# MPF-Optimization-Laboratory/ConicIP.jl

Hardware: NVIDIA B200
Metric: kkt_factor_plus_solves_per_sec (higher is better)
Workload: dtype f64

## Files before the change

conicip.jl_b200/csrc/engine.h:

```cpp
#pragma once
#include <vector>

#include "../../include/conicip_b200.h"
#include "kernels.cuh"

constexpr int NV = 8;
constexpr int MV = 10;
constexpr int PV = 6;

namespace cip {
struct Multi;

struct RowStructure {
  bool on = false;
  int nsing = 0, nempty = 0, nr = 0, nr_pad = 0, nJ = 0, nJ_pad = 0;
  bool compressed = false, base_has_gtg = false, fold = false;
  double *At4r = nullptr, *Atil4r = nullptr, *Hr4 = nullptr;
  double* Base4 = nullptr;
  GemmOperand map{};
  int *rest_row = nullptr, *J = nullptr, *Jinv = nullptr;
  int* row_code = nullptr;
  int *sing_ptr = nullptr, *sing_row = nullptr, *sing_col = nullptr;
  double* sing_val = nullptr;
  ConeDesc cd{};
  int *d_type = nullptr, *d_off = nullptr, *d_rowcone = nullptr, *d_qlist = nullptr, *d_slist = nullptr;
  int* cone_map = nullptr;
  Scaling Fi{};
  double *xr[2] = {}, *yJ[2] = {}, *outr[2] = {}, *outJ[2] = {};

  struct Split {
    bool on = false;
    int nK = 0, nK_pad = 0, from_rest = 0, from_Q = 0, from_G = 0;
    bool g_in_D = false;
    bool factored = false;
    std::vector<int> K;
    std::vector<char> q_couple;
    struct QEntry { int i, j; double v; };
    std::vector<QEntry> qtrip;
    int *dK = nullptr, *Kpos = nullptr, *JK = nullptr;
    double *QK4 = nullptr, *BaseK4 = nullptr, *HK4 = nullptr, *WinvK = nullptr;
    double *qD = nullptr, *hD = nullptr, *kscale = nullptr;
    double *GK4 = nullptr, *ZK4 = nullptr;
    CholPlan chol{};
    GemmOperand mapZK{}, mapG{};
    int* fail = nullptr;
    double* kv[2][3] = {};
  } sp;
};

struct FastSyrk {
  bool on = false;
  int depth = 0;
  int leaf = 0;
  int K2 = 0;
  unsigned two = 0;
  int nchunk = 0;
  int* colexp = nullptr;
  double* colss = nullptr;
  double* M = nullptr;
  double* M2 = nullptr;
  int4* table = nullptr;
};
}

struct cip_engine {
  cip::Multi* multi = nullptr;
  cip::Multi* parent = nullptr;
  int shard_index = 0;
  bool always_sync = false;
  int n = 0, m = 0, p = 0, n_pad = 0, m_pad = 0, p_pad = 0, ncones = 0;
  int device = 0;
  cudaStream_t stream = nullptr, own_stream = nullptr;
  cip_options opt{};
  double *At4 = nullptr, *Atil4 = nullptr, *Qq4 = nullptr, *H4 = nullptr, *Winv = nullptr;
  double *G4 = nullptr, *Z4 = nullptr, *S4 = nullptr, *Sbase4 = nullptr, *WinvS = nullptr;
  cip::GemmOperand mapAtil{}, mapZ{};
  cip::CholPlan cholH{}, cholS{};
  int* info = nullptr;
  std::vector<int> h_type, h_off;
  int *d_type = nullptr, *d_off = nullptr, *d_rowcone = nullptr, *d_qlist = nullptr, *d_slist = nullptr;
  int *d_sord = nullptr, *d_roff = nullptr;
  double* d_sws = nullptr;
  std::vector<int> h_slist, h_sord, h_roff;
  size_t r_total = 0;
  cip::ConeDesc cd{};
  cip::Scaling F{}, Fi{};
  bool have_scaling = false, have_factor = false;
  double* gemm_ws = nullptr;
  bool fold = false;
  cip::GemmOperand mapAt{};
  int aug_rows = 0;
  double aug_rho = 0.0;
  cip::RowStructure rs;
  cip::FastSyrk fast;
  std::vector<void*> owned;
  double* nv[NV] = {};
  double* mv[MV] = {};
  double* pv[PV] = {};
  double* nv2[6] = {};
  double* mv2[6] = {};
  double* pv2[5] = {};
  double* partial = nullptr;
  int partial_cap = 0;
  double* scalar = nullptr;
  void* comm = nullptr;
  int nranks = 1, rank = 0;
  double* Hp = nullptr;
  cudaStream_t cs = nullptr, s2 = nullptr;
  cudaEvent_t evc[16] = {};
  cip_stats_t st{};
  cudaEvent_t ev[8] = {};
  size_t bytes = 0;
  bool need_sync = false;
};


namespace cip {
int engine_allreduce(cip_engine* h, double* buf, size_t count);
int engine_create_single(cip_handle* out, int n, int m, int p, const double* Q, int ldq, const double* A, int lda,
                         const double* G, int ldg, const cip_csc* Qs, const cip_csc* As, const cip_csc* Gs,
                         int ncones, const int* cone_type, const int* cone_dim, const cip_options* opts);
const char* last_error_string();
int engine_decide_fold(cip_engine* h, bool can, size_t mn, bool* fold);
int engine_setup_comm(cip_engine* h);

int fast_syrk_plan(cip_engine* h, bool can);
size_t fast_syrk_atil_doubles(const cip_engine* h);
int fast_syrk_setup(cip_engine* h);
int fast_syrk_drop(cip_engine* h);
int fast_syrk_form(cip_engine* h, const double* cin);

int structure_build_dense(cip_engine* h);
int structure_build_csc(cip_engine* h, const cip_csc* A);
int structure_finish(cip_engine* h);
int structure_form_H(cip_engine* h);
int structure_AT(cip_engine* h, double* out, const double* x, const double* add, int b);
int structure_AT2(cip_engine* h, double* outa, double* outb, const double* xa, const double* xb, const double* adda,
                  const double* addb);
int structure_A(cip_engine* h, double* out, const double* y, int b);
int structure_A2(cip_engine* h, double* outa, double* outb, const double* ya, const double* yb);
int split_classify_csc_Q(cip_engine* h, const cip_csc* Q);
int split_diag_Q(cip_engine* h, const double* q);
int split_build(cip_engine* h);
int split_factor(cip_engine* h);
int split_add_delta(cip_engine* h, double delta);
int split_solve(cip_engine* h, double** nv, double** pv, int b, bool schur);
int split_mul_Q(cip_engine* h, double* y, const double* x);
int split_get_H(cip_engine* h, double* tmp);

int multi_create(cip_handle* out, int n, int m, int p, const double* Q, int ldq, const double* A, int lda,
                 const double* G, int ldg, const cip_csc* Qs, const cip_csc* As, const cip_csc* Gs, int ncones,
                 const int* cone_type, const int* cone_dim, const cip_options* opts);
int multi_destroy(cip_engine* h);
int multi_factor(cip_engine* h, const int* kind, const double* fa, const double* fb, const double* fD,
                 const double* fR, int factor);
int multi_get_scaling(cip_engine* h, int* kind, double* fa, double* fb, double* fD, double* fR);
int multi_nt_scaling(cip_engine* h, const double* v, const double* s, double* lambda_out, int factor);
int multi_solve(cip_engine* h, const double* ry, const double* rw, const double* rv, double* dy, double* dw,
                double* dv);
int multi_solve_multi(cip_engine* h, int nrhs, const double* ry, int ldy, const double* rw, int ldw, const double* rv,
                      int ldv, double* dy, double* dw, double* dv);
int multi_apply(cip_engine* h, int op, const double* x, double* y);
int multi_maxstep(cip_engine* h, const double* x, const double* d, double d_scale, double* alpha_out);
int multi_prod_div(cip_engine* h, const double* x, const double* y, double* o, int divide);
int multi_mul_A(cip_engine* h, int trans, const double* x, double* y);
int multi_mul_GQ(cip_engine* h, int which, int trans, const double* x, double* y);
int multi_ipm_solve(cip_engine* h, const double* c, const double* b, const double* d, const cip_ipm_options* opts,
                    double* y, double* w, double* v, cip_ipm_result* result);
int multi_stats(cip_engine* h, cip_stats_t* out);
int multi_simple(cip_engine* h, int what, double* out, int ldo);
void multi_barrier(cip::Multi* m);
}
```

conicip.jl_b200/csrc/fast_syrk.cu:

```cuda
#include <stdlib.h>

#include <algorithm>
#include <vector>

#include "engine.h"

namespace cip {

namespace {

constexpr int FAST_SYRK_LEAF = 2048;
constexpr int FAST_SYRK_N0 = 12288;
constexpr int FAST_SYRK_L2_MIN = 1024;

struct SumsArgs {
  int h, kqh, pstride, count;
  int a_row, a_kq, b_row, b_kq, s_row, s_kq, t_row, t_kq;
  int scale_a, scale_b;
};

__device__ __forceinline__ void winograd_sums(double* __restrict__ X, int ld, const SumsArgs& s,
                                              const int* __restrict__ colexp) {
  const int kq = blockIdx.x;
  const int x = blockIdx.y * blockDim.x + threadIdx.x;
  if (x >= s.count) return;
  const int h = s.h, KQ2 = s.kqh;
  const int p = x / h, i = x - p * h, base = p * s.pstride;
  const int xa = base + s.a_row + i, xb = base + s.b_row + i;
  const int ka = s.a_kq + kq, kb = s.b_kq + kq;
  auto at = [&](int kqq, int r) { return reinterpret_cast<double2*>(X + ((size_t)kqq * ld + r) * 4); };
  auto ld4 = [&](int kqq, int r, double f, double2& lo, double2& hi) {
    const double2* q = at(kqq, r);
    lo = q[0]; hi = q[1];
    lo.x *= f; lo.y *= f; hi.x *= f; hi.y *= f;
  };
  auto fac = [&](int on, int r) { return on ? ldexp(1.0, -colexp[r]) : 1.0; };
  const double fa1 = fac(s.scale_a, xa), fa2 = fac(s.scale_a, xa + h);
  const double fb1 = fac(s.scale_b, xb), fb2 = fac(s.scale_b, xb + h);
  double2 a11l, a11h, a12l, a12h, a21l, a21h, a22l, a22h, b11l, b11h, b12l, b12h, b21l, b21h, b22l, b22h;
  ld4(ka, xa, fa1, a11l, a11h);
  ld4(ka + KQ2, xa, fa1, a12l, a12h);
  ld4(ka, xa + h, fa2, a21l, a21h);
  ld4(ka + KQ2, xa + h, fa2, a22l, a22h);
  ld4(kb, xb, fb1, b11l, b11h);
  ld4(kb + KQ2, xb, fb1, b12l, b12h);
  ld4(kb, xb + h, fb2, b21l, b21h);
  ld4(kb + KQ2, xb + h, fb2, b22l, b22h);
  auto add = [](double2 u, double2 v) { return make_double2(u.x + v.x, u.y + v.y); };
  auto sub = [](double2 u, double2 v) { return make_double2(u.x - v.x, u.y - v.y); };
  const double2 s1l = add(a21l, a22l), s1h = add(a21h, a22h);
  const double2 s2l = sub(s1l, a11l), s2h = sub(s1h, a11h);
  const double2 s3l = sub(a11l, a21l), s3h = sub(a11h, a21h);
  const double2 s4l = sub(a12l, s2l), s4h = sub(a12h, s2h);
  const double2 t1l = sub(b21l, b11l), t1h = sub(b21h, b11h);
  const double2 t2l = sub(b22l, t1l), t2h = sub(b22h, t1h);
  const double2 t3l = sub(b22l, b21l), t3h = sub(b22h, b21h);
  const double2 t4l = sub(t2l, b12l), t4h = sub(t2h, b12h);
  const int ks = s.s_kq + kq, kt = s.t_kq + kq, rs = base + s.s_row + i, rt = base + s.t_row + i;
  auto st4 = [&](int kqq, int r, double2 lo, double2 hi) { double2* q = at(kqq, r); q[0] = lo; q[1] = hi; };
  st4(ks, rs, s1l, s1h);
  st4(ks, rs + h, s2l, s2h);
  st4(ks, rs + 2 * h, s3l, s3h);
  st4(ks, rs + 3 * h, s4l, s4h);
  st4(kt, rt, t1l, t1h);
  st4(kt, rt + h, t2l, t2h);
  st4(kt, rt + 2 * h, t3l, t3h);
  st4(kt, rt + 3 * h, t4l, t4h);
}

__global__ void __launch_bounds__(256)
winograd_sums_kernel(double* __restrict__ X, int ld, const SumsArgs s, const int* __restrict__ colexp) {
  winograd_sums(X, ld, s, colexp);
}
__global__ void __launch_bounds__(256)
winograd_sums2_kernel(double* __restrict__ X, int ld, const SumsArgs s, const int* __restrict__ colexp) {
  winograd_sums(X, ld, s, colexp);
}

__global__ void __launch_bounds__(256)
winograd_combine2_kernel(const double* __restrict__ M2, double* __restrict__ M, int h2, int q, int pstride,
                         int x_row, int y_row, int raw_x, int raw_y, const int* __restrict__ colexp) {
  const int nt2 = h2 / TILE, G2 = nt2 * nt2, nt = 2 * nt2, G = nt * nt;
  const int L2 = blockIdx.x, p = blockIdx.y;
  const int ti = L2 % nt2, tj = L2 / nt2;
  const int xr = p * pstride + x_row, yr = p * pstride + y_row;
  const size_t slab = (size_t)TILE * TILE;
  const double* Mp = M2 + ((size_t)p * 7 * G2 + L2) * slab;
  double* Mq = M + (size_t)(p * 7 + q) * G * slab;
  for (int e = threadIdx.x * 2; e < TILE * TILE; e += 512) {
    const int quad = e / (TILE * 4), lr = (e % (TILE * 4)) >> 2, c = e & 3;
    const int i = ti * TILE + lr, j = tj * TILE + quad * 4 + c;
    double2 P[7];
#pragma unroll
    for (int r = 0; r < 7; ++r) P[r] = *reinterpret_cast<const double2*>(Mp + (size_t)r * G2 * slab + e);
    const int ex1 = raw_x ? colexp[xr + i] : 0, ex2 = raw_x ? colexp[xr + h2 + i] : 0;
    const int ey1[2] = {raw_y ? colexp[yr + j] : 0, raw_y ? colexp[yr + j + 1] : 0};
    const int ey2[2] = {raw_y ? colexp[yr + h2 + j] : 0, raw_y ? colexp[yr + h2 + j + 1] : 0};
    double o[4][2];
#pragma unroll
    for (int k = 0; k < 2; ++k) {
      const double p1 = k ? P[0].y : P[0].x, p2 = k ? P[1].y : P[1].x, p3 = k ? P[2].y : P[2].x;
      const double p4 = k ? P[3].y : P[3].x, p5 = k ? P[4].y : P[4].x, p6 = k ? P[5].y : P[5].x;
      const double p7 = k ? P[6].y : P[6].x;
      const double s1 = ldexp(p1, -(ex1 + ey1[k])), s2 = ldexp(p2, -(ex1 + ey1[k]));
      const double u2 = s1 + p6;
      const double u3 = u2 + p7, u4 = u2 + p5;
      o[0][k] = s1 + s2;
      o[1][k] = u4 + ldexp(p3, -ey2[k]);
      o[2][k] = u3 - ldexp(p4, -ex2);
      o[3][k] = u3 + p5;
    }
#pragma unroll
    for (int b = 0; b < 4; ++b) {
      const int L = (ti + (b >> 1) * nt2) + (tj + (b & 1) * nt2) * nt;
      *reinterpret_cast<double2*>(Mq + (size_t)L * slab + e) = make_double2(o[b][0], o[b][1]);
    }
  }
}

__global__ void __launch_bounds__(256)
winograd_combine_kernel(const double* __restrict__ M, const double* __restrict__ Cin, double* __restrict__ H, int ld,
                        int h, int scaled, const int* __restrict__ colexp) {
  const int nt = h / TILE, G = nt * nt;
  const int L = blockIdx.x, p = blockIdx.y;
  const int ti = L % nt, tj = L / nt;
  const int ra = 4 * p * h, rb = ra + 2 * h;
  const size_t slab = (size_t)TILE * TILE;
  const double* Mp = M + ((size_t)p * 7 * G + L) * slab;
  for (int e = threadIdx.x * 2; e < TILE * TILE; e += 512) {
    const int quad = e / (TILE * 4), lr = (e % (TILE * 4)) >> 2, c = e & 3;
    const int i = ti * TILE + lr, j = tj * TILE + quad * 4 + c;
    double2 P[7];
#pragma unroll
    for (int q = 0; q < 7; ++q) P[q] = *reinterpret_cast<const double2*>(Mp + (size_t)q * G * slab + e);
    const int eb1 = colexp[rb + i], eb2 = colexp[rb + h + i];
    const int ea1[2] = {colexp[ra + j], colexp[ra + j + 1]};
    const int ea2[2] = {colexp[ra + h + j], colexp[ra + h + j + 1]};
    double o[4][2];
#pragma unroll
    for (int k = 0; k < 2; ++k) {
      const double p1 = k ? P[0].y : P[0].x, p2 = k ? P[1].y : P[1].x, p3 = k ? P[2].y : P[2].x;
      const double p4 = k ? P[3].y : P[3].x, p5 = k ? P[4].y : P[4].x, p6 = k ? P[5].y : P[5].x;
      const double p7 = k ? P[6].y : P[6].x;
      const double u2 = (scaled ? p1 : ldexp(p1, -(eb1 + ea1[k]))) + p6;
      const double u3 = u2 + p7, u4 = u2 + p5;
      o[0][k] = scaled ? ldexp(p1 + p2, eb1 + ea1[k]) : p1 + p2;
      o[1][k] = ldexp(u4 + (scaled ? p3 : ldexp(p3, -ea2[k])), eb1 + ea2[k]);
      o[2][k] = ldexp(u3 - (scaled ? p4 : ldexp(p4, -eb2)), eb2 + ea1[k]);
      o[3][k] = ldexp(u3 + p5, eb2 + ea2[k]);
    }
#pragma unroll
    for (int b = 0; b < 4; ++b) {
      const size_t idx = q4_index(rb + (b >> 1) * h + i, ra + (b & 1) * h + j, ld);
      double2 v = make_double2(o[b][0], o[b][1]);
      if (Cin) {
        const double2 q = *reinterpret_cast<const double2*>(Cin + idx);
        v.x += q.x;
        v.y += q.y;
      }
      *reinterpret_cast<double2*>(H + idx) = v;
    }
  }
}

int env_int(const char* name, int dflt) {
  const char* e = getenv(name);
  return (e && *e) ? atoi(e) : dflt;
}

template <typename T>
int falloc(cip_engine* h, T** p, size_t count) {
  *p = nullptr;
  if (count == 0) count = 1;
  CIP_CUDA(cudaMalloc(reinterpret_cast<void**>(p), count * sizeof(T)));
  CIP_CUDA(cudaMemsetAsync(*p, 0, count * sizeof(T), h->stream));
  h->bytes += count * sizeof(T);
  h->owned.push_back(*p);
  return 0;
}

size_t m_doubles(int n_pad) { return (size_t)7 * n_pad / 4 * n_pad / 4; }

size_t m2_doubles(int n_pad, unsigned two) {
  if (!two) return 0;
  int d = 0;
  while (!(two >> d & 1u)) ++d;
  const size_t h2 = (size_t)n_pad >> (d + 3);
  return (size_t)7 * ((size_t)1 << d) * h2 * h2;
}

size_t atil_rows(const FastSyrk& f) { return (size_t)4 * f.K2 + (f.two ? f.K2 / 2 : 0); }

void winograd_ops(int4 ops[7], int xr, int xk, int yr, int yk, int hh, int kqh, int sr, int sk, int tr, int tk) {
  ops[0] = make_int4(xr, xk, yr, yk);
  ops[1] = make_int4(xr, xk + kqh, yr, yk + kqh);
  ops[2] = make_int4(sr + 3 * hh, sk, yr + hh, yk + kqh);
  ops[3] = make_int4(xr + hh, xk + kqh, tr + 3 * hh, tk);
  ops[4] = make_int4(sr, sk, tr, tk);
  ops[5] = make_int4(sr + hh, sk, tr + hh, tk);
  ops[6] = make_int4(sr + 2 * hh, sk, tr + 2 * hh, tk);
}

void level1_ops(int4 ops[7], int p, int hh, int KQ2) {
  const int ra = 4 * p * hh, rb = ra + 2 * hh;
  winograd_ops(ops, rb, 0, ra, 0, hh, KQ2, ra, 2 * KQ2, ra, 3 * KQ2);
}

void level2_ops(int4 ops[7], int4 o, int p, int hh, int KQ2) {
  const int ra = 4 * p * hh;
  winograd_ops(ops, o.x, o.y, o.z, o.w, hh / 2, KQ2 / 2, ra, 4 * KQ2, ra + 2 * hh, 4 * KQ2);
}

}

int fast_syrk_plan(cip_engine* h, bool can) {
  FastSyrk& f = h->fast;
  f = FastSyrk{};
  const int mode = env_int("CIP_FAST_SYRK", 2);
  if (!can || mode == 0 || h->m_pad == 0) return 0;
  int leaf = std::max(256, env_int("CIP_FAST_SYRK_LEAF", FAST_SYRK_LEAF));
  if (mode == 1) leaf = std::min(leaf, h->n_pad / 2);
  int W = h->n_pad, depth = 0;
  while (W % 512 == 0 && W / 2 >= leaf) { W /= 2; ++depth; }
  if (depth == 0 || (mode != 1 && h->n_pad < FAST_SYRK_N0)) return 0;
  const int levels = env_int("CIP_FAST_SYRK_LEVELS", 0);
  unsigned two = 0;
  for (int d = 0; d < depth && levels != 1; ++d) {
    const int h2 = h->n_pad >> (d + 3);
    if (h2 % TILE == 0 && (h2 >= FAST_SYRK_L2_MIN || levels == 2)) two |= 1u << d;
  }
  const size_t nn = (size_t)h->n_pad * h->n_pad;
  const size_t colss = (size_t)scale_panel_norms_chunks(h->m_pad) * h->n_pad;
  for (;; two = 0) {
    f.two = two;
    f.K2 = round_up(h->m_pad, two ? 128 : 64) / 2;
    if (mode == 1) break;
    size_t free_b = 0, total_b = 0;
    CIP_CUDA(cudaMemGetInfo(&free_b, &total_b));
    const size_t need = (atil_rows(f) * h->n_pad + m_doubles(h->n_pad) + m2_doubles(h->n_pad, two) + colss + 3 * nn +
                         (size_t)GEMM_WS_DOUBLES) * 8 + (size_t(1) << 30);
    if (free_b >= need) break;
    if (!two) { f = FastSyrk{}; return 0; }
  }
  f.on = true;
  f.depth = depth;
  f.leaf = W;
  f.nchunk = scale_panel_norms_chunks(h->m_pad);
  return 0;
}

size_t fast_syrk_atil_doubles(const cip_engine* h) { return atil_rows(h->fast) * h->n_pad; }

int fast_syrk_setup(cip_engine* h) {
  FastSyrk& f = h->fast;
  if (!f.on) return 0;
  CIP_TRY(falloc(h, &f.colexp, h->n_pad));
  CIP_TRY(falloc(h, &f.colss, (size_t)f.nchunk * h->n_pad));
  CIP_TRY(falloc(h, &f.M, m_doubles(h->n_pad)));
  if (f.two) CIP_TRY(falloc(h, &f.M2, m2_doubles(h->n_pad, f.two)));
  const int KQ2 = f.K2 / 4;
  std::vector<int4> t;
  for (int l = 0; l < (1 << f.depth); ++l) {
    const int r0 = l * f.leaf;
    t.push_back(make_int4(r0, 0, r0, 0));
    t.push_back(make_int4(r0, r0, 0, 0));
  }
  int4 ops[7], sub[7];
  for (int d = 0; d < f.depth; ++d) {
    const int hh = h->n_pad >> (d + 2);
    for (int p = 0; p < (1 << d); ++p) {
      level1_ops(ops, p, hh, KQ2);
      for (const int4& o : ops) {
        t.push_back(o);
        t.push_back(make_int4(0, 0, 0, 0));
      }
    }
  }
  for (int d = 0; d < f.depth; ++d) {
    if (!(f.two >> d & 1u)) continue;
    const int hh = h->n_pad >> (d + 2);
    for (int q = 0; q < 7; ++q)
      for (int p = 0; p < (1 << d); ++p) {
        level1_ops(ops, p, hh, KQ2);
        level2_ops(sub, ops[q], p, hh, KQ2);
        for (const int4& o : sub) {
          t.push_back(o);
          t.push_back(make_int4(0, 0, 0, 0));
        }
      }
  }
  CIP_TRY(falloc(h, &f.table, t.size()));
  CIP_CUDA(cudaMemcpyAsync(f.table, t.data(), t.size() * sizeof(int4), cudaMemcpyHostToDevice, h->stream));
  CIP_CUDA(cudaStreamSynchronize(h->stream));
  return 0;
}

int fast_syrk_drop(cip_engine* h) {
  FastSyrk& f = h->fast;
  if (!f.on) return 0;
  CIP_CUDA(cudaStreamSynchronize(h->stream));
  for (void* p : {(void*)f.colexp, (void*)f.colss, (void*)f.M, (void*)f.M2, (void*)f.table}) {
    if (!p) continue;
    h->owned.erase(std::find(h->owned.begin(), h->owned.end(), p));
    CIP_CUDA(cudaFree(p));
  }
  CIP_CUDA(cudaFree(h->Atil4));
  h->bytes -= fast_syrk_atil_doubles(h) * 8;
  const size_t mn = (size_t)h->m_pad * h->n_pad;
  CIP_CUDA(cudaMalloc(reinterpret_cast<void**>(&h->Atil4), mn * 8));
  CIP_CUDA(cudaMemsetAsync(h->Atil4, 0, mn * 8, h->stream));
  h->bytes += mn * 8;
  CIP_TRY(make_q4_tensor_map(&h->mapAtil.map, h->Atil4, h->n_pad, h->m_pad / 4));
  f = FastSyrk{};
  return 0;
}

int fast_syrk_form(cip_engine* h, const double* cin) {
  const FastSyrk& f = h->fast;
  cudaStream_t s = h->stream;
  const int KQ2 = f.K2 / 4, L = 1 << f.depth;
  int sub_entry = L + 7 * (L - 1);
  for (int d = 0; d < f.depth; ++d) {
    const int pairs = 1 << d, hh = h->n_pad >> (d + 2), nt = hh / TILE;
    const bool two = f.two >> d & 1u;
    SumsArgs sa{hh, KQ2, 4 * hh, pairs * hh, 2 * hh, 0, 0, 0, 0, 2 * KQ2, 0, 3 * KQ2, 1, 1};
    winograd_sums_kernel<<<dim3(KQ2, (sa.count + 255) / 256), 256, 0, s>>>(h->Atil4, h->n_pad, sa, f.colexp);
    CIP_CHECK_LAUNCH();
    GemmArgs g{};
    g.lower = 0; g.ntm = g.ntn = nt; g.sym = 0;
    g.nk = f.K2 / 32;
    g.Ctm = f.M; g.ldc = h->n_pad; g.alpha = 1.0;
    g.ws = h->gemm_ws; g.ws_doubles = GEMM_WS_DOUBLES;
    g.group = f.table + 2 * (L + 7 * (pairs - 1));
    g.group_tiles = nt * nt;
    g.tile_count = 7 * pairs * nt * nt;
    if (!two) {
      CIP_TRY(launch_gemm_nt(h->mapAtil, h->mapAtil, g, s));
    } else {
      const int h2 = hh / 2, nt2 = h2 / TILE;
      int4 ops[7];
      level1_ops(ops, 0, hh, KQ2);
      for (int q = 0; q < 7; ++q) {
        const int4 o = ops[q];
        const int raw_x = o.y < 2 * KQ2, raw_y = o.w < 2 * KQ2;
        SumsArgs s2{h2, KQ2 / 2, 4 * hh, pairs * h2, o.x, o.y, o.z, o.w, 0, 4 * KQ2, 2 * hh, 4 * KQ2, raw_x, raw_y};
        winograd_sums2_kernel<<<dim3(KQ2 / 2, (s2.count + 255) / 256), 256, 0, s>>>(h->Atil4, h->n_pad, s2, f.colexp);
        CIP_CHECK_LAUNCH();
        GemmArgs g2 = g;
        g2.ntm = g2.ntn = nt2;
        g2.nk = f.K2 / 64;
        g2.Ctm = f.M2;
        g2.group = f.table + 2 * sub_entry;
        g2.group_tiles = nt2 * nt2;
        g2.tile_count = 7 * pairs * nt2 * nt2;
        sub_entry += 7 * pairs;
        CIP_TRY(launch_gemm_nt(h->mapAtil, h->mapAtil, g2, s));
        winograd_combine2_kernel<<<dim3(nt2 * nt2, pairs), 256, 0, s>>>(f.M2, f.M, h2, q, 4 * hh, o.x, o.z, raw_x,
                                                                        raw_y, f.colexp);
        CIP_CHECK_LAUNCH();
      }
    }
    winograd_combine_kernel<<<dim3(nt * nt, pairs), 256, 0, s>>>(f.M, cin, h->H4, h->n_pad, hh, two, f.colexp);
    CIP_CHECK_LAUNCH();
  }
  const int T = f.leaf / TILE;
  GemmArgs a{};
  a.lower = 1; a.ntm = a.ntn = T; a.sym = 1;
  a.nk = h->m_pad / 32;
  a.Cin = cin; a.Cout = h->H4; a.ldc = h->n_pad; a.alpha = 1.0;
  a.ws = h->gemm_ws; a.ws_doubles = GEMM_WS_DOUBLES;
  a.group = f.table;
  a.group_tiles = T * (T + 1) / 2;
  a.tile_count = L * a.group_tiles;
  CIP_TRY(launch_gemm_nt(h->mapAtil, h->mapAtil, a, s));
  return 0;
}

}
```

Baseline: 0.5816.

## Generalize Winograd fast SYRK to recursive multi-level Strassen-Winograd expansion

Replaces the fixed one-or-two-level Winograd scheme in the fast SYRK path with a recursive expansion that supports up to three levels per depth. It adds per-level scratch buffers, generalized operand tables, and row offsets for the sum buffers. The aim is to cut the O(n^3) GEMM flops further for large KKT matrices. In exchange it adds more sum and combine kernel launches, extra memory, and possible floating-point error growth in f64.

```diff
diff --git a/conicip.jl_b200/csrc/engine.h b/conicip.jl_b200/csrc/engine.h
--- a/conicip.jl_b200/csrc/engine.h
+++ b/conicip.jl_b200/csrc/engine.h
@@ -48,17 +48,18 @@
   } sp;
 };
 
+constexpr int FAST_SYRK_MAX_LEVELS = 3;
 struct FastSyrk {
   bool on = false;
   int depth = 0;
   int leaf = 0;
   int K2 = 0;
-  unsigned two = 0;
+  int levels[32] = {};
+  int max_levels = 1;
   int nchunk = 0;
   int* colexp = nullptr;
   double* colss = nullptr;
-  double* M = nullptr;
-  double* M2 = nullptr;
+  double* M[FAST_SYRK_MAX_LEVELS] = {};
   int4* table = nullptr;
 };
 }
diff --git a/conicip.jl_b200/csrc/fast_syrk.cu b/conicip.jl_b200/csrc/fast_syrk.cu
--- a/conicip.jl_b200/csrc/fast_syrk.cu
+++ b/conicip.jl_b200/csrc/fast_syrk.cu
@@ -76,10 +76,14 @@
 winograd_sums2_kernel(double* __restrict__ X, int ld, const SumsArgs s, const int* __restrict__ colexp) {
   winograd_sums(X, ld, s, colexp);
 }
-
-__global__ void __launch_bounds__(256)
-winograd_combine2_kernel(const double* __restrict__ M2, double* __restrict__ M, int h2, int q, int pstride,
-                         int x_row, int y_row, int raw_x, int raw_y, const int* __restrict__ colexp) {
+__global__ void __launch_bounds__(256)
+winograd_sums3_kernel(double* __restrict__ X, int ld, const SumsArgs s, const int* __restrict__ colexp) {
+  winograd_sums(X, ld, s, colexp);
+}
+
+__device__ __forceinline__ void winograd_combine_sub(const double* __restrict__ M2, double* __restrict__ M, int h2,
+                                                     int q, int pstride, int x_row, int y_row, int raw_x, int raw_y,
+                                                     const int* __restrict__ colexp) {
   const int nt2 = h2 / TILE, G2 = nt2 * nt2, nt = 2 * nt2, G = nt * nt;
   const int L2 = blockIdx.x, p = blockIdx.y;
   const int ti = L2 % nt2, tj = L2 / nt2;
@@ -116,6 +120,17 @@
       *reinterpret_cast<double2*>(Mq + (size_t)L * slab + e) = make_double2(o[b][0], o[b][1]);
     }
   }
+}
+
+__global__ void __launch_bounds__(256)
+winograd_combine2_kernel(const double* __restrict__ M2, double* __restrict__ M, int h2, int q, int pstride,
+                         int x_row, int y_row, int raw_x, int raw_y, const int* __restrict__ colexp) {
+  winograd_combine_sub(M2, M, h2, q, pstride, x_row, y_row, raw_x, raw_y, colexp);
+}
+__global__ void __launch_bounds__(256)
+winograd_combine3_kernel(const double* __restrict__ M2, double* __restrict__ M, int h2, int q, int pstride,
+                         int x_row, int y_row, int raw_x, int raw_y, const int* __restrict__ colexp) {
+  winograd_combine_sub(M2, M, h2, q, pstride, x_row, y_row, raw_x, raw_y, colexp);
 }
 
 __global__ void __launch_bounds__(256)
@@ -181,15 +196,18 @@
 
 size_t m_doubles(int n_pad) { return (size_t)7 * n_pad / 4 * n_pad / 4; }
 
-size_t m2_doubles(int n_pad, unsigned two) {
-  if (!two) return 0;
-  int d = 0;
-  while (!(two >> d & 1u)) ++d;
-  const size_t h2 = (size_t)n_pad >> (d + 3);
-  return (size_t)7 * ((size_t)1 << d) * h2 * h2;
-}
-
-size_t atil_rows(const FastSyrk& f) { return (size_t)4 * f.K2 + (f.two ? f.K2 / 2 : 0); }
+size_t mk_doubles(const FastSyrk& f, int n_pad, int k) {
+  for (int d = 0; d < f.depth; ++d) {
+    if (f.levels[d] < k) continue;
+    const size_t hk = (size_t)n_pad >> (d + k + 1);
+    return (size_t)7 * ((size_t)1 << d) * hk * hk;
+  }
+  return 0;
+}
+
+size_t atil_rows(const FastSyrk& f) { return (size_t)4 * f.K2 + (f.K2 - (f.K2 >> (f.max_levels - 1))); }
+
+int sums_kq(int k, int KQ2) { return 4 * KQ2 + KQ2 - (KQ2 >> (k - 2)); }
 
 void winograd_ops(int4 ops[7], int xr, int xk, int yr, int yk, int hh, int kqh, int sr, int sk, int tr, int tk) {
   ops[0] = make_int4(xr, xk, yr, yk);
@@ -206,9 +224,63 @@
   winograd_ops(ops, rb, 0, ra, 0, hh, KQ2, ra, 2 * KQ2, ra, 3 * KQ2);
 }
 
-void level2_ops(int4 ops[7], int4 o, int p, int hh, int KQ2) {
-  const int ra = 4 * p * hh;
-  winograd_ops(ops, o.x, o.y, o.z, o.w, hh / 2, KQ2 / 2, ra, 4 * KQ2, ra + 2 * hh, 4 * KQ2);
+void level_ops(int4 ops[7], int4 o, int k, int p, int hh, int KQ2) {
+  const int ra = 4 * p * hh, sk = sums_kq(k, KQ2);
+  winograd_ops(ops, o.x, o.y, o.z, o.w, hh >> (k - 1), KQ2 >> (k - 1), ra, sk, ra + 2 * hh, sk);
+}
+
+void push_deepest(std::vector<int4>& t, int4 o, int k, int levels, int pairs, int hh, int KQ2) {
+  int4 sub[7];
+  level_ops(sub, o, k + 1, 0, hh, KQ2);
+  if (k + 1 < levels) {
+    for (const int4& s : sub) push_deepest(t, s, k + 1, levels, pairs, hh, KQ2);
+    return;
+  }
+  for (int p = 0; p < pairs; ++p)
+    for (const int4& s : sub) {
+      t.push_back(make_int4(s.x + 4 * p * hh, s.y, s.z + 4 * p * hh, s.w));
+      t.push_back(make_int4(0, 0, 0, 0));
+    }
+}
+
+struct DepthRun {
+  cip_engine* h;
+  int hh, pairs, KQ2, levels;
+  GemmArgs g;
+  int entry;
+};
+
+int expand(DepthRun& c, int k, int4 o, int slot) {
+  const FastSyrk& f = c.h->fast;
+  cudaStream_t s = c.h->stream;
+  const int hs = c.hh >> k, nts = hs / TILE, sk = sums_kq(k + 1, c.KQ2);
+  const int raw_x = o.y < 2 * c.KQ2, raw_y = o.w < 2 * c.KQ2;
+  const bool deepest = k + 1 >= std::min(c.levels, FAST_SYRK_MAX_LEVELS);
+  SumsArgs sa{hs, c.KQ2 >> k, 4 * c.hh, c.pairs * hs, o.x, o.y, o.z, o.w, 0, sk, 2 * c.hh, sk, raw_x, raw_y};
+  const dim3 sg(sa.kqh, (sa.count + 255) / 256);
+  (k == 1 ? winograd_sums2_kernel : winograd_sums3_kernel)<<<sg, 256, 0, s>>>(c.h->Atil4, c.h->n_pad, sa, f.colexp);
+  CIP_CHECK_LAUNCH();
+  if (deepest) {
+    GemmArgs g = c.g;
+    g.ntm = g.ntn = nts;
+    g.nk = (f.K2 >> k) / 32;
+    g.Ctm = f.M[k];
+    g.group = f.table + 2 * c.entry;
+    g.group_tiles = nts * nts;
+    g.tile_count = 7 * c.pairs * nts * nts;
+    c.entry += 7 * c.pairs;
+    CIP_TRY(launch_gemm_nt(c.h->mapAtil, c.h->mapAtil, g, s));
+  } else {
+    int4 sub[7];
+    level_ops(sub, o, k + 1, 0, c.hh, c.KQ2);
+    for (int r = 0; r < 7; ++r) CIP_TRY(expand(c, k + 1, sub[r], r));
+  }
+  const dim3 cg(nts * nts, c.pairs);
+  const int rx = deepest && raw_x, ry = deepest && raw_y;
+  (k == 1 ? winograd_combine2_kernel : winograd_combine3_kernel)<<<cg, 256, 0, s>>>(f.M[k], f.M[k - 1], hs, slot,
+                                                                                     4 * c.hh, o.x, o.z, rx, ry, f.colexp);
+  CIP_CHECK_LAUNCH();
+  return 0;
 }
 
 }
@@ -223,27 +295,32 @@
   int W = h->n_pad, depth = 0;
   while (W % 512 == 0 && W / 2 >= leaf) { W /= 2; ++depth; }
   if (depth == 0 || (mode != 1 && h->n_pad < FAST_SYRK_N0)) return 0;
-  const int levels = env_int("CIP_FAST_SYRK_LEVELS", 0);
-  unsigned two = 0;
-  for (int d = 0; d < depth && levels != 1; ++d) {
-    const int h2 = h->n_pad >> (d + 3);
-    if (h2 % TILE == 0 && (h2 >= FAST_SYRK_L2_MIN || levels == 2)) two |= 1u << d;
+  const int force = env_int("CIP_FAST_SYRK_LEVELS", 0);
+  const int cap = force >= 1 ? std::min(force, FAST_SYRK_MAX_LEVELS) : FAST_SYRK_MAX_LEVELS;
+  f.depth = depth;
+  for (int d = 0; d < depth; ++d) {
+    int k = 1;
+    for (; k < cap; ++k) {
+      const int hk = h->n_pad >> (d + k + 2);
+      if (hk % TILE != 0 || (hk < FAST_SYRK_L2_MIN && force < 1)) break;
+    }
+    f.levels[d] = k;
   }
   const size_t nn = (size_t)h->n_pad * h->n_pad;
   const size_t colss = (size_t)scale_panel_norms_chunks(h->m_pad) * h->n_pad;
-  for (;; two = 0) {
-    f.two = two;
-    f.K2 = round_up(h->m_pad, two ? 128 : 64) / 2;
+  for (;;) {
+    f.max_levels = *std::max_element(f.levels, f.levels + depth);
+    f.K2 = round_up(h->m_pad, 64 << (f.max_levels - 1)) / 2;
     if (mode == 1) break;
     size_t free_b = 0, total_b = 0;
     CIP_CUDA(cudaMemGetInfo(&free_b, &total_b));
-    const size_t need = (atil_rows(f) * h->n_pad + m_doubles(h->n_pad) + m2_doubles(h->n_pad, two) + colss + 3 * nn +
-                         (size_t)GEMM_WS_DOUBLES) * 8 + (size_t(1) << 30);
-    if (free_b >= need) break;
-    if (!two) { f = FastSyrk{}; return 0; }
+    size_t need = atil_rows(f) * h->n_pad + m_doubles(h->n_pad) + colss + 3 * nn + (size_t)GEMM_WS_DOUBLES;
+    for (int k = 2; k <= f.max_levels; ++k) need += mk_doubles(f, h->n_pad, k);
+    if (free_b >= need * 8 + (size_t(1) << 30)) break;
+    if (f.max_levels == 1) { f = FastSyrk{}; return 0; }
+    for (int d = 0; d < depth; ++d) f.levels[d] = std::min(f.levels[d], f.max_levels - 1);
   }
   f.on = true;
-  f.depth = depth;
   f.leaf = W;
   f.nchunk = scale_panel_norms_chunks(h->m_pad);
   return 0;
@@ -256,8 +333,8 @@
   if (!f.on) return 0;
   CIP_TRY(falloc(h, &f.colexp, h->n_pad));
   CIP_TRY(falloc(h, &f.colss, (size_t)f.nchunk * h->n_pad));
-  CIP_TRY(falloc(h, &f.M, m_doubles(h->n_pad)));
-  if (f.two) CIP_TRY(falloc(h, &f.M2, m2_doubles(h->n_pad, f.two)));
+  CIP_TRY(falloc(h, &f.M[0], m_doubles(h->n_pad)));
+  for (int k = 2; k <= f.max_levels; ++k) CIP_TRY(falloc(h, &f.M[k - 1], mk_doubles(f, h->n_pad, k)));
   const int KQ2 = f.K2 / 4;
   std::vector<int4> t;
   for (int l = 0; l < (1 << f.depth); ++l) {
@@ -265,7 +342,7 @@
     t.push_back(make_int4(r0, 0, r0, 0));
     t.push_back(make_int4(r0, r0, 0, 0));
   }
-  int4 ops[7], sub[7];
+  int4 ops[7];
   for (int d = 0; d < f.depth; ++d) {
     const int hh = h->n_pad >> (d + 2);
     for (int p = 0; p < (1 << d); ++p) {
@@ -277,17 +354,10 @@
     }
   }
   for (int d = 0; d < f.depth; ++d) {
-    if (!(f.two >> d & 1u)) continue;
+    if (f.levels[d] < 2) continue;
     const int hh = h->n_pad >> (d + 2);
-    for (int q = 0; q < 7; ++q)
-      for (int p = 0; p < (1 << d); ++p) {
-        level1_ops(ops, p, hh, KQ2);
-        level2_ops(sub, ops[q], p, hh, KQ2);
-        for (const int4& o : sub) {
-          t.push_back(o);
-          t.push_back(make_int4(0, 0, 0, 0));
-        }
-      }
+    level1_ops(ops, 0, hh, KQ2);
+    for (const int4& o : ops) push_deepest(t, o, 1, f.levels[d], 1 << d, hh, KQ2);
   }
   CIP_TRY(falloc(h, &f.table, t.size()));
   CIP_CUDA(cudaMemcpyAsync(f.table, t.data(), t.size() * sizeof(int4), cudaMemcpyHostToDevice, h->stream));
@@ -299,7 +369,7 @@
   FastSyrk& f = h->fast;
   if (!f.on) return 0;
   CIP_CUDA(cudaStreamSynchronize(h->stream));
-  for (void* p : {(void*)f.colexp, (void*)f.colss, (void*)f.M, (void*)f.M2, (void*)f.table}) {
+  for (void* p : {(void*)f.colexp, (void*)f.colss, (void*)f.M[0], (void*)f.M[1], (void*)f.M[2], (void*)f.table}) {
     if (!p) continue;
     h->owned.erase(std::find(h->owned.begin(), h->owned.end(), p));
     CIP_CUDA(cudaFree(p));
@@ -322,45 +392,28 @@
   int sub_entry = L + 7 * (L - 1);
   for (int d = 0; d < f.depth; ++d) {
     const int pairs = 1 << d, hh = h->n_pad >> (d + 2), nt = hh / TILE;
-    const bool two = f.two >> d & 1u;
     SumsArgs sa{hh, KQ2, 4 * hh, pairs * hh, 2 * hh, 0, 0, 0, 0, 2 * KQ2, 0, 3 * KQ2, 1, 1};
     winograd_sums_kernel<<<dim3(KQ2, (sa.count + 255) / 256), 256, 0, s>>>(h->Atil4, h->n_pad, sa, f.colexp);
     CIP_CHECK_LAUNCH();
     GemmArgs g{};
     g.lower = 0; g.ntm = g.ntn = nt; g.sym = 0;
     g.nk = f.K2 / 32;
-    g.Ctm = f.M; g.ldc = h->n_pad; g.alpha = 1.0;
+    g.Ctm = f.M[0]; g.ldc = h->n_pad; g.alpha = 1.0;
     g.ws = h->gemm_ws; g.ws_doubles = GEMM_WS_DOUBLES;
     g.group = f.table + 2 * (L + 7 * (pairs - 1));
     g.group_tiles = nt * nt;
     g.tile_count = 7 * pairs * nt * nt;
-    if (!two) {
+    if (f.levels[d] == 1) {
       CIP_TRY(launch_gemm_nt(h->mapAtil, h->mapAtil, g, s));
     } else {
-      const int h2 = hh / 2, nt2 = h2 / TILE;
+      DepthRun run{h, hh, pairs, KQ2, f.levels[d], g, sub_entry};
       int4 ops[7];
       level1_ops(ops, 0, hh, KQ2);
-      for (int q = 0; q < 7; ++q) {
-        const int4 o = ops[q];
-        const int raw_x = o.y < 2 * KQ2, raw_y = o.w < 2 * KQ2;
-        SumsArgs s2{h2, KQ2 / 2, 4 * hh, pairs * h2, o.x, o.y, o.z, o.w, 0, 4 * KQ2, 2 * hh, 4 * KQ2, raw_x, raw_y};
-        winograd_sums2_kernel<<<dim3(KQ2 / 2, (s2.count + 255) / 256), 256, 0, s>>>(h->Atil4, h->n_pad, s2, f.colexp);
-        CIP_CHECK_LAUNCH();
-        GemmArgs g2 = g;
-        g2.ntm = g2.ntn = nt2;
-        g2.nk = f.K2 / 64;
-        g2.Ctm = f.M2;
-        g2.group = f.table + 2 * sub_entry;
-        g2.group_tiles = nt2 * nt2;
-        g2.tile_count = 7 * pairs * nt2 * nt2;
-        sub_entry += 7 * pairs;
-        CIP_TRY(launch_gemm_nt(h->mapAtil, h->mapAtil, g2, s));
-        winograd_combine2_kernel<<<dim3(nt2 * nt2, pairs), 256, 0, s>>>(f.M2, f.M, h2, q, 4 * hh, o.x, o.z, raw_x,
-                                                                        raw_y, f.colexp);
-        CIP_CHECK_LAUNCH();
-      }
-    }
-    winograd_combine_kernel<<<dim3(nt * nt, pairs), 256, 0, s>>>(f.M, cin, h->H4, h->n_pad, hh, two, f.colexp);
+      for (int q = 0; q < 7; ++q) CIP_TRY(expand(run, 1, ops[q], q));
+      sub_entry = run.entry;
+    }
+    winograd_combine_kernel<<<dim3(nt * nt, pairs), 256, 0, s>>>(f.M[0], cin, h->H4, h->n_pad, hh, f.levels[d] > 1,
+                                                                 f.colexp);
     CIP_CHECK_LAUNCH();
   }
   const int T = f.leaf / TILE;
```

Result: faster. 0.5986, median of 6 (+2.9%).
